# huangzh13/StyleGAN.pytorch

Measured on AMD Instinct MI355X. Metric: img/s full G+D train step, 1024x1024 depth-9 bf16, higher is better.
Workload: dtype bf16; 1 GPU; ffhq1024: StyleGAN 1024x1024, progressive depth index 8, logistic+R1, alpha 0.5, batch 4/GPU, global batch 4; global_batch=4, parallelism=dp1

## Files before the change

include/sgx.h:

```cpp
#ifndef SGX_H
#define SGX_H
#include <stddef.h>
#include <stdint.h>
#ifdef __cplusplus
extern "C" {
#endif

enum { SGX_F32 = 0, SGX_BF16 = 1 };
enum { SGX_ACT_NONE = 0, SGX_ACT_LRELU = 1, SGX_ACT_RELU = 2 };
enum { SGX_EINVAL = -1, SGX_EUNSUPPORTED = -2, SGX_EWORKSPACE = -3 };

int sgx_version(void);
const char* sgx_last_error(void);
int sgx_clear_error(void);
int sgx_stream_wait_stream(void* waiter, void* signaler);
int sgx_selftest_tr16(void* out256, void* stream);

int sgx_prof_start(int mode, int only_of);
int sgx_prof_count(void);
int sgx_prof_get(int i, char* name, int name_cap, float* ms, double* flops, double* bytes, char* desc, int desc_cap);
int sgx_prof_get_launch(int i, unsigned* grid3, unsigned* block3, size_t* lds);

int sgx_conv3x3(const void* x, const void* w, const float* bias, void* y, int B, int H, int W, int Cin, int Cout,
                int act, const void* mask, int dtype, void* stream);
int sgx_conv4x4s2_down(const void* x, const void* w, const float* bias, void* y, int B, int H, int W, int Cin,
                       int Cout, int act, int dtype, void* stream);
int sgx_conv4x4s2_up(const void* x, const void* w, void* y, int B, int H, int W, int Cin, int Cout, int dtype,
                     void* stream);
int sgx_conv_variant(int geo, const void* x, const void* w, const float* bias, void* y, int B, int H, int W, int Cin, int Cout,
                     int act, int dtype, int variant, void* stream);
size_t sgx_conv_splitk_ws_bytes(int geo, int B, int H, int W, int Cin, int Cout, int dtype);
int sgx_conv_splitk(int geo, const void* x, const void* w, const float* bias, void* y, const void* mask, int B, int H, int W, int Cin, int Cout,
                    int act, int dtype, void* ws, size_t ws_bytes, void* stream);

int sgx_conv_config(int geo, int B, int H, int W, int Cin, int Cout, int dtype, int* cfg5);
enum { SGX_PACK_S = 0, SGX_PACK_D = 1, SGX_PACK_U = 2, SGX_PACK_UF = 3 };
int sgx_pack_weight(const float* w, void* fwd, void* adj, int O, int I, int Ipad, int mode, float scale, int dtype,
                    void* stream);
#define SGX_PACK_ROW 10
int sgx_pack_weight_blocks(int O, int Ipad);
int sgx_pack_weight_multi(const void* table, int n, int total_blocks, int dtype, void* stream);
size_t sgx_wgrad_ws_bytes(int taps, int B, int H, int W, int Ck, int Cn);
#define SGX_WGRAD_PLAN_INTS 11
int sgx_wgrad_plan(int taps, int B, int H, int W, int Ck, int Cn, int dtype, size_t ws_bytes, int* out);
int sgx_wgrad3x3_param(const void* x, const void* dy, float* dW, float* db, void* ws, size_t ws_bytes, int B, int H, int W,
                       int Cx, int Cdy, int adjoint, float scale, int O, int I, int accumulate, int dtype, void* stream);
int sgx_wgrad4x4s2_param(const void* fine, const void* coarse, float* dW, float* db, void* ws, size_t ws_bytes, int B, int H,
                         int W, int Cfine, int Ccoarse, int mode, float scale, int O, int I, int accumulate, int dtype,
                         void* stream);

int sgx_bias_act(const void* x, const float* bias, float bscale, void* y, size_t npix, int C, int act, int dtype,
                 void* stream);
int sgx_lrelu_bwd(const void* dy, const void* y, void* dx, size_t n, float slope, float scale, const float* scale_dev, int dtype,
                  void* stream);
int sgx_lrelu_bwd_bits(const void* dy, const void* bits, void* dx, size_t n, float slope, float scale, const float* scale_dev, int dtype,
                       void* stream);
int sgx_conv4x4s2_down_fade_ok(int B, int H, int W, int Cin, int Cout, int dtype);
int sgx_conv4x4s2_down_fade(const void* x, const void* w, const float* bias, const void* resid, float alpha, float beta, const float* ab_dev,
                            void* y, void* bits, int B, int H, int W, int Cin, int Cout, int dtype, void* stream);
int sgx_conv4x4s2_down_fade_rgb(const void* x, const void* w, const float* bias, const float* pimg, const float* wr, float ws, const float* rb,
                                float bs1, float bs2, float alpha, float beta, const float* ab_dev, void* y, void* bits, int B, int H, int W,
                                int Cin, int Cout, int dtype, void* stream);
size_t sgx_fade_rgb_bwd_ws_bytes(size_t npix, int C);
int sgx_fade_rgb_bwd(const void* g, const void* bits, const float* pimg, const float* wr, float ws, float bs, float alpha, float beta,
                     const float* ab_dev, void* gy, float* dwr, float* drb, int acc, float* gpimg, void* wsbuf, size_t ws_bytes, size_t npix, int C,
                     int dtype, void* stream);
int sgx_fade_rgb_bwd_finish(const void* wsbuf, size_t ws_bytes, size_t npix, int C, float ws, float bs, float beta, const float* ab_dev,
                            float* dwr, float* drb, int acc, void* stream);
int sgx_fade_rgb_bwd2(const void* ggy, const float* ggp, const void* bits, const float* wr, float ws, float alpha, float beta, const float* ab_dev,
                      void* out, size_t npix, int C, int dtype, void* stream);
int sgx_axpby(const void* a, const void* b, void* out, float alpha, float beta, size_t n, int dtype, void* stream);
int sgx_axpby_dev(const void* a, const void* b, void* out, const float* alpha_dev, const float* beta_dev, size_t n, int dtype,
                  void* stream);
int sgx_blur3x3(const void* x, void* y, int B, int H, int W, int C, int dtype, void* stream);
int sgx_blur3x3_act(const void* x, const void* z, void* y, int B, int H, int W, int C, int mode, int dtype, void* stream);
int sgx_blur3x3_bits(const void* x, const void* bits, void* y, int B, int H, int W, int C, int mode, int dtype, void* stream);
int sgx_blur_kxk(const void* x, void* y, const float* taps_host, int K, int pad, int B, int IH, int IW, int OH, int OW, int C,
                 int dtype, void* stream);
int sgx_images_u8_to_nhwc(const void* src, void* dst, const int* flip, int B, int H, int W, int src_chw, int dtype, void* stream);
int sgx_pool2(const void* x, void* y, int B, int H, int W, int C, float scale, int dtype, void* stream);
int sgx_up2(const void* x, void* y, int B, int H, int W, int C, float scale, int dtype, void* stream);
int sgx_up2_add(const void* x, const void* a, void* y, int B, int H, int W, int C, float scale, int dtype, void* stream);
size_t sgx_colsum_ws_bytes(size_t npix, int C);
int sgx_colsum(const void* x, float* out, float scale, void* ws, size_t ws_bytes, size_t npix, int C, int dtype,
               void* stream);

int sgx_rgb_in(const float* img, const float* w, int sj, int sc, float wscale, const float* bias, void* y, size_t npix,
               int C, int dtype, void* stream);
int sgx_rgb_out(const void* x, const float* w, int sj, int sc, float wscale, const float* bias, float* img, size_t npix,
                int C, int dtype, void* stream);
int sgx_rgb_in_add(const float* img, const float* w, int sj, int sc, float wscale, const void* add, void* y, size_t npix, int C, int dtype,
                   void* stream);
size_t sgx_rgb_wgrad_ws_bytes(size_t npix, int C);
int sgx_img_in(const float* img, const float* w, int J, int sj, int sc, float wscale, const float* bias, void* y, size_t npix, int C, int dtype,
               void* stream);
int sgx_img_out(const void* x, const float* w, int J, int sj, int sc, float wscale, const float* bias, float* img, size_t npix, int C, int dtype,
                void* stream);
size_t sgx_img_wgrad_ws_bytes(size_t npix, int J, int C);
int sgx_img_wgrad(const float* img, const void* f, float* dw, int J, int sj, int sc, float wscale, void* ws, size_t ws_bytes, size_t npix, int C,
                  int dtype, void* stream);
int sgx_images_u8_to_nhwc_c(const void* src, void* dst, const int* flip, int B, int H, int W, int J, int src_chw, int dtype, void* stream);
int sgx_downsample_fade_rgb(const float* x, float* out, int B, int H, int W, float alpha, float beta, const float* ab_dev, void* stream);
size_t sgx_diffaug_ws_bytes(int B, int H, int W);
int sgx_diffaug(const float* x, float* y, const float* u, int B, int H, int W, int policy_bits, int adjoint, int with_bias, void* ws,
                size_t ws_bytes, void* stream);
int sgx_ada_gates(const float* gu, const float* state, int policy_bits, int* img_bits, int B, void* stream);
int sgx_diffaug_gated(const float* x, float* y, const float* u, const int* img_bits, int B, int H, int W, int policy_bits, int adjoint,
                      int with_bias, void* ws, size_t ws_bytes, void* stream);
int sgx_ada_update(const float* real_logits, int B, float* state, float target, float adjust_per_image, int interval, void* stream);
int sgx_diffaug_blit(const float* x, float* y, const float* u, int u_stride, const int* img_bits, int B, int H, int W, int policy_bits,
                     int adjoint, int with_bias, void* ws, size_t ws_bytes, void* stream);
int sgx_ada_gates_n(const float* gu, int gu_stride, int n_ops, const float* state, int policy_bits, int* img_bits, int B, void* stream);
int sgx_ada_geom_matrix(const float* u, int u_stride, const float* gu, int gu_stride, const float* state, int policy_bits, float* mat, int B,
                        void* stream);
int sgx_ada_geom(const float* x, float* y, const float* mat, int B, int H, int W, int adjoint, void* stream);
int sgx_ada_geom_reflect(const float* x, float* y, const float* mat, int B, int H, int W, int adjoint, void* stream);
#define SGX_ADA_GEOM_REFLECT_PLAN_INTS 6
int sgx_ada_geom_reflect_plan(int B, int H, int W, int adjoint, int aligned, int* out);
int sgx_ada_color_matrix(const float* u, int u_stride, const float* gu, int gu_stride, const float* state, int policy_bits, float* mat, int B,
                         void* stream);
int sgx_ada_color(const float* x, float* y, const float* mat, int B, int H, int W, int adjoint, int with_bias, void* stream);
int sgx_ada_filter_matrix(const float* u, int u_stride, const float* gu, int gu_stride, const float* state, int policy_bits, float* mat, int B,
                          void* stream);
size_t sgx_ada_filter_workspace_bytes(int B, int H, int W);
int sgx_ada_filter(const float* x, float* y, const float* mat, int B, int H, int W, int adjoint, void* ws, size_t ws_bytes, void* stream);
#define SGX_ADA_FILTER_PLAN_INTS 13
int sgx_ada_filter_plan(int B, int H, int W, int adjoint, int aligned, int* out);
int sgx_ada_corrupt_table(const float* u, int u_stride, const float* gu, int gu_stride, const float* state, int policy_bits, int H, int W,
                          float* tab, int B, void* stream);
int sgx_ada_corrupt(const float* x, float* y, const float* tab, int B, int H, int W, int mode, void* stream);
#define SGX_ADA_CORRUPT_PLAN_INTS 5
int sgx_ada_corrupt_plan(int B, int H, int W, int mode, int aligned, int* out);
// ... 102 lines not shown
```

stylegan/pytorch_amd/functional.py:

```python
import contextlib
import functools
import os
import weakref
from collections import namedtuple

import numpy as np
import torch
from torch.autograd import Function
from torch.autograd.function import once_differentiable

from . import native as N

_DATA_GRAD_ONLY = 0


@contextlib.contextmanager
def data_grad_only():
    global _DATA_GRAD_ONLY
    _DATA_GRAD_ONLY += 1
    try:
        yield
    finally:
        _DATA_GRAD_ONLY -= 1

# ... 221 lines not shown
            ent[4][2].add(raw)
    if got is None:
        w = _c(weight.detach())
        if w.dtype != torch.float32:
            raise N.SgxError("parameters must be fp32")
        O, I = w.shape[0], w.shape[1]
        fwd, adj = _pack_alloc(w, sub)
        N.check(N.lib().sgx_pack_weight(N.ptr(w), N.ptr(fwd), N.ptr(adj), O, I, ipad, MODES[mode], float(scale),
                                        N.F32 if dtype == torch.float32 else N.BF16, N.stream()), "sgx_pack_weight")
        got = (fwd, adj)
        ent[2][sub] = got
        ent[4] = _pack_mark()
    return got


def clear_pack_cache():
    for ent in _PACKS.values():
        ent[1], ent[2] = None, {}
    _UPBLUR_PACKS.clear()


_UPBLUR_PACKS = {}


def upblur_pack(weight, mode, scale, ipad, adjoint):
    key = (id(weight), mode, float(scale), int(ipad), bool(adjoint))
    tag = _pack_tag(weight)
    ent = _UPBLUR_PACKS.get(key)
    if ent is not None and ent[0]() is weight and ent[1] == tag:
        raw = N.stream()
        if raw not in ent[3][2] or (not _FAST_FORK and raw != ent[3][1]):
            _stream_of(raw).wait_event(ent[3][0])
            ent[3][2].add(raw)
        return ent[2]
    w = _c(weight.detach())
    if w.dtype != torch.float32 or int(ipad) != w.shape[1]:
        raise N.SgxError("conv+blur composite pack: contiguous fp32 parameter without channel padding expected")
    O, I = w.shape[0], w.shape[1]
    Nn, K = (I, O) if adjoint else (O, I)
    wc = torch.empty(((9 * 4 + 22 * 2) * Nn * K,), dtype=torch.bfloat16, device=w.device)
    N.check(N.lib().sgx_pack_upblur(N.ptr(w), N.ptr(wc), O, I, MODES[mode], int(bool(adjoint)), float(scale) / 16.0, N.stream()), "sgx_pack_upblur")
    _UPBLUR_PACKS[key] = [weakref.ref(weight, lambda _r, k=key: _UPBLUR_PACKS.pop(k, None)), tag, wc, _pack_mark()]
    return wc


@functools.lru_cache(maxsize=None)
def _splitk_ws_bytes(gi, B, H, W, Cin, Cout, dt):
    return int(N.lib().sgx_conv_splitk_ws_bytes(gi, B, H, W, Cin, Cout, dt))


def _conv_launch(geo, x, wq, bias, act, mask=None):
    B, H, W, Cin = x.shape
    taps, Cout, K = wq.shape
    if K != Cin:
        raise N.SgxError(f"conv: weight pack expects {K} input channels, activation has {Cin}")
    L = N.lib()
    gi = "SDU".index(geo)
    wsb = _splitk_ws_bytes(gi, B, H, W, Cin, Cout, N.dt(x))
    if wsb:
        oh, ow = (H, W) if geo == "S" else ((H // 2, W // 2) if geo == "D" else (2 * H, 2 * W))
        y = torch.empty((B, oh, ow, Cout), dtype=x.dtype, device=x.device)
        if mask is not None and (geo != "S" or mask.shape != y.shape or mask.dtype != y.dtype):
            raise N.SgxError("conv: the output mask must have the output's shape and dtype (3x3 geometry)")
        ws = N.workspace(wsb, x.device)
        N.check(L.sgx_conv_splitk(gi, N.ptr(x), N.ptr(wq), N.ptr(bias), N.ptr(y), N.ptr(mask), B, H, W, Cin, Cout, act, N.dt(x), N.ptr(ws), wsb, N.stream()),
                "sgx_conv_splitk")
        return y
    if geo == "S":
        y = torch.empty((B, H, W, Cout), dtype=x.dtype, device=x.device)
        if mask is not None and (mask.shape != y.shape or mask.dtype != y.dtype):
            raise N.SgxError("conv: the output mask must have the output's shape and dtype")
        N.check(L.sgx_conv3x3(N.ptr(x), N.ptr(wq), N.ptr(bias), N.ptr(y), B, H, W, Cin, Cout, act, N.ptr(mask), N.dt(x), N.stream()), "sgx_conv3x3")
    elif geo == "D":
        assert mask is None
        y = torch.empty((B, H // 2, W // 2, Cout), dtype=x.dtype, device=x.device)
        N.check(L.sgx_conv4x4s2_down(N.ptr(x), N.ptr(wq), N.ptr(bias), N.ptr(y), B, H, W, Cin, Cout, act, N.dt(x), N.stream()), "sgx_conv4x4s2_down")
    else:
        assert bias is None and act == 0 and mask is None
        y = torch.empty((B, 2 * H, 2 * W, Cout), dtype=x.dtype, device=x.device)
        N.check(L.sgx_conv4x4s2_up(N.ptr(x), N.ptr(wq), N.ptr(y), B, H, W, Cin, Cout, N.dt(x), N.stream()), "sgx_conv4x4s2_up")
    return y


def _wgrad_param(mode, adjoint, x, gy, weight, scale, want_bias=False, into=None):
    L = N.lib()
    O, I = weight.shape[0], weight.shape[1]
    acc_w = into is not None and into[0] is not None
    acc_b = want_bias and into is not None and into[1] is not None
    dW = into[0] if acc_w else torch.empty((O, I, 3, 3), dtype=torch.float32, device=x.device)
    db = (into[1] if acc_b else torch.empty((O,), dtype=torch.float32, device=x.device)) if want_bias else None
    acc = (1 if acc_w else 0) | (2 if acc_b else 0)
    B = x.shape[0]
    if mode == "S":
        _, H, W, Cx = x.shape
        Cdy = gy.shape[3]
        wsb = L.sgx_wgrad_ws_bytes(9, B, H, W, Cx, Cdy)
        ws = N.workspace(wsb, x.device)
        N.check(L.sgx_wgrad3x3_param(N.ptr(x), N.ptr(gy), N.ptr(dW), N.ptr(db), N.ptr(ws), wsb, B, H, W, Cx, Cdy, int(adjoint),
                                     float(scale), O, I, acc, N.dt(x), N.stream()), "sgx_wgrad3x3_param")
        return dW, db
    launched = ADJ_GEO[mode] if adjoint else FWD_GEO[mode]
    fine, coarse = (x, gy) if launched == "D" else (gy, x)
    _, H, W, Cf = fine.shape
    Cc = coarse.shape[3]
    wsb = L.sgx_wgrad_ws_bytes(16, B, H, W, Cf, Cc)
    ws = N.workspace(wsb, x.device)
    N.check(L.sgx_wgrad4x4s2_param(N.ptr(fine), N.ptr(coarse), N.ptr(dW), N.ptr(db), N.ptr(ws), wsb, B, H, W, Cf, Cc, MODES[mode],
                                   float(scale), O, I, acc, N.dt(x), N.stream()), "sgx_wgrad4x4s2_param")
    return dW, db


class ConvFn(Function):

    @staticmethod
    def forward(ctx, x, weight, bias, mode, scale, ipad, adjoint, act, mask=None, defer_act=False, x_masked=False, stats=None,
                x_pre=None, bits_out=False, x_pre_bits=None):
        x = _c(x)
        fwd, adj = packs(weight, mode, scale, ipad, x.dtype)
        geo = ADJ_GEO[mode] if adjoint else FWD_GEO[mode]
        ctx.cfg = (mode, scale, ipad, adjoint, act, bias is not None, bool(defer_act), bool(x_masked))
        ctx.bias_ref = weakref.ref(bias) if bias is not None else (lambda: None)
        ctx.set_materialize_grads(False)
        if bits_out:
            assert geo == "S" and not adjoint and stats is None
            y, bits = _conv_bits_launch(x, fwd, None if bias is None else _c(bias.detach()), act, mask)
            ctx.mark_non_differentiable(bits)
            ctx.save_for_backward(x, weight, y if (act and not defer_act) else None, mask, x_pre, x_pre_bits)
            return y, bits
        if stats is not None:
            assert geo == "S" and not adjoint and bias is None and act == 0 and mask is None
            y, part = _conv_stats_launch(x, fwd, *stats)
            ctx.mark_non_differentiable(part)
            ctx.save_for_backward(x, weight, None, None, x_pre, x_pre_bits)
            return y, part
        y = _conv_launch(geo, x, adj if adjoint else fwd, None if bias is None else _c(bias.detach()), act, mask)
        ctx.save_for_backward(x, weight, y if (act and not defer_act) else None, mask, x_pre, x_pre_bits)
        return y

    @staticmethod
    def backward(ctx, gy, _gpart=None):
        if gy is None:
            return (None,) * 15
        x, weight, y, mask, x_pre, xb = ctx.saved_tensors[:6]
        mode, scale, ipad, adjoint, act, has_bias, defer_act, x_masked = ctx.cfg
        gy = _c(gy)
        if mask is not None:
            gy = _bcall(LReluBwdFn, gy, mask, 0.2, 1.0)
        if act and not defer_act:
            gy = _bcall(LReluBwdFn, gy, y, 0.2, 1.0)
        gx = gw = gb = None
        if ctx.needs_input_grad[0]:
            if x_pre is not None or xb is not None:
                assert not x_masked
                cout_b = weight.shape[1] if not adjoint else weight.shape[0]
                if xb is not None and conv_upblur_ok(gy, cout_b, mode, not adjoint):
                    gx = _bcall(ConvBlurFn, gy, weight, mode, scale, ipad, not adjoint, None, xb)
                elif x_pre is not None and conv_blur_ok(gy, cout_b, mode, not adjoint, has_mask_tensor=True):
                    gx = _bcall(ConvBlurFn, gy, weight, mode, scale, ipad, not adjoint, x_pre)
                else:
                    gx = _bcall(BlurMaskFn, _bcall(ConvFn, gy, weight, None, mode, scale, ipad, not adjoint, 0), x_pre, xb)
            else:
                gx = _bcall(ConvFn, gy, weight, None, mode, scale, ipad, not adjoint, 0, x if x_masked else None, False, False)
        if not _DATA_GRAD_ONLY:
            want_b = has_bias and ctx.needs_input_grad[2]
            fuse_b = want_b and ctx.needs_input_grad[1] and not adjoint and mode in ("S", "D")
            if ctx.needs_input_grad[1] and _ACCUM_PARAM_GRADS and weight.is_leaf and not torch.is_grad_enabled():
                bias = ctx.bias_ref() if fuse_b else None
                if fuse_b and (bias is None or not bias.is_leaf):
                    fuse_b, bias = False, None
                dW, db = _param_grads(mode, adjoint, _c(x), gy, weight, scale, fuse_b, (weight.grad, bias.grad if fuse_b else None))
                if weight.grad is None:
                    weight.grad = dW
                if fuse_b:
                    if bias.grad is None:
                        bias.grad = db
                    want_b = False
                if GRAD_NOTE is not None:
                    GRAD_NOTE(weight)
                    if fuse_b:
                        GRAD_NOTE(bias)
            elif ctx.needs_input_grad[1]:
                gw, gb = _bcall(WgradFn, x, gy, weight, mode, scale, adjoint, fuse_b)
            if want_b and not fuse_b:
                gb = _bcall(ColSumFn, gy, 1.0)
        return gx, gw, gb, None, None, None, None, None, None, None, None, None, None, None, None


# ... 1985 lines not shown
```

stylegan/pytorch_amd/native.py:

```python
import ctypes
import os
import subprocess
import threading

import torch

_HERE = os.path.dirname(os.path.abspath(__file__))
LIB_PATH = os.environ.get("SGX_HIP_LIB") or os.path.join(_HERE, "libsgx_hip.so")
CSRC = os.path.join(_HERE, "csrc")

F32, BF16 = 0, 1
ACT_NONE, ACT_LRELU, ACT_RELU = 0, 1, 2
EPI_ACT, EPI_NORM = 1, 2
PACK_S, PACK_D, PACK_U, PACK_UF = 0, 1, 2, 3

_lib = None
_lock = threading.Lock()

c_void_p, c_int, c_float, c_size_t = ctypes.c_void_p, ctypes.c_int, ctypes.c_float, ctypes.c_size_t
P, I, F, Z = c_void_p, c_int, c_float, c_size_t

SIGNATURES = {
    "sgx_version": (I, []),
    "sgx_last_error": (ctypes.c_char_p, []),
    "sgx_clear_error": (I, []),
    "sgx_stream_wait_stream": (I, [P, P]),
    "sgx_conv3x3": (I, [P, P, P, P, I, I, I, I, I, I, P, I, P]),
    "sgx_conv_variant": (I, [I, P, P, P, P, I, I, I, I, I, I, I, I, P]),
    "sgx_conv4x4s2_down": (I, [P, P, P, P, I, I, I, I, I, I, I, P]),
    "sgx_conv4x4s2_up": (I, [P, P, P, I, I, I, I, I, I, P]),
    "sgx_wgrad_ws_bytes": (Z, [I, I, I, I, I, I]),
    "sgx_wgrad_plan": (I, [I, I, I, I, I, I, I, Z, P]),
    "sgx_images_u8_to_nhwc": (I, [P, P, P, I, I, I, I, I, P]),
    "sgx_selftest_tr16": (I, [P, P]),
    "sgx_conv_splitk_ws_bytes": (Z, [I, I, I, I, I, I, I]),
    "sgx_conv_splitk": (I, [I, P, P, P, P, P, I, I, I, I, I, I, I, P, Z, P]),
    "sgx_conv_config": (I, [I, I, I, I, I, I, I, P]),
    "sgx_prof_start": (I, [I, I]),
    "sgx_prof_count": (I, []),
    "sgx_prof_get": (I, [I, P, I, P, P, P, P, I]),
    "sgx_prof_get_launch": (I, [I, P, P, P]),
    "sgx_pack_weight": (I, [P, P, P, I, I, I, I, F, I, P]),
    "sgx_pack_weight_multi": (I, [P, I, I, I, P]),
    "sgx_pack_weight_blocks": (I, [I, I]),
    "sgx_wgrad3x3_param": (I, [P, P, P, P, P, Z, I, I, I, I, I, I, F, I, I, I, I, P]),
    "sgx_wgrad4x4s2_param": (I, [P, P, P, P, P, Z, I, I, I, I, I, I, F, I, I, I, I, P]),
    "sgx_bias_act": (I, [P, P, F, P, Z, I, I, I, P]),
    "sgx_lrelu_bwd": (I, [P, P, P, Z, F, F, P, I, P]),
    "sgx_lrelu_bwd_bits": (I, [P, P, P, Z, F, F, P, I, P]),
    "sgx_conv4x4s2_down_fade_ok": (I, [I, I, I, I, I, I]),
    "sgx_conv4x4s2_down_fade": (I, [P, P, P, P, F, F, P, P, P, I, I, I, I, I, I, P]),
    "sgx_conv4x4s2_down_fade_rgb": (I, [P, P, P, P, P, F, P, F, F, F, F, P, P, P, I, I, I, I, I, I, P]),
    "sgx_fade_rgb_bwd_ws_bytes": (Z, [Z, I]),
    "sgx_fade_rgb_bwd": (I, [P, P, P, P, F, F, F, F, P, P, P, P, I, P, P, Z, Z, I, I, P]),
    "sgx_fade_rgb_bwd_finish": (I, [P, Z, Z, I, F, F, F, P, P, P, I, P]),
    "sgx_fade_rgb_bwd2": (I, [P, P, P, P, F, F, F, P, P, Z, I, I, P]),
    "sgx_axpby": (I, [P, P, P, F, F, Z, I, P]),
    "sgx_axpby_dev": (I, [P, P, P, P, P, Z, I, P]),
    "sgx_blur3x3": (I, [P, P, I, I, I, I, I, P]),
    "sgx_blur3x3_act": (I, [P, P, P, I, I, I, I, I, I, P]),
    "sgx_blur_kxk": (I, [P, P, P, I, I, I, I, I, I, I, I, I, P]),
    "sgx_pool2": (I, [P, P, I, I, I, I, F, I, P]),
    "sgx_up2": (I, [P, P, I, I, I, I, F, I, P]),
    "sgx_up2_add": (I, [P, P, P, I, I, I, I, F, I, P]),
    "sgx_colsum_ws_bytes": (Z, [Z, I]),
    "sgx_colsum": (I, [P, P, F, P, Z, Z, I, I, P]),
    "sgx_rgb_in": (I, [P, P, I, I, F, P, P, Z, I, I, P]),
    "sgx_rgb_in_add": (I, [P, P, I, I, F, P, P, Z, I, I, P]),
    "sgx_rgb_out": (I, [P, P, I, I, F, P, P, Z, I, I, P]),
    "sgx_img_in": (I, [P, P, I, I, I, F, P, P, Z, I, I, P]),
    "sgx_img_out": (I, [P, P, I, I, I, F, P, P, Z, I, I, P]),
    "sgx_img_wgrad_ws_bytes": (Z, [Z, I, I]),
    "sgx_img_wgrad": (I, [P, P, P, I, I, I, F, P, Z, Z, I, I, P]),
    "sgx_images_u8_to_nhwc_c": (I, [P, P, P, I, I, I, I, I, I, P]),
    "sgx_downsample_fade_rgb": (I, [P, P, I, I, I, F, F, P, P]),
    "sgx_diffaug_ws_bytes": (Z, [I, I, I]),
    "sgx_diffaug": (I, [P, P, P, I, I, I, I, I, I, P, Z, P]),
    "sgx_ada_gates": (I, [P, P, I, P, I, P]),
    "sgx_diffaug_gated": (I, [P, P, P, P, I, I, I, I, I, I, P, Z, P]),
    "sgx_ada_update": (I, [P, I, P, F, F, I, P]),
    "sgx_diffaug_blit": (I, [P, P, P, I, P, I, I, I, I, I, I, P, Z, P]),
    "sgx_ada_gates_n": (I, [P, I, I, P, I, P, I, P]),
    "sgx_ada_geom_matrix": (I, [P, I, P, I, P, I, P, I, P]),
    "sgx_ada_geom": (I, [P, P, P, I, I, I, I, P]),
    "sgx_ada_geom_reflect": (I, [P, P, P, I, I, I, I, P]),
    "sgx_ada_geom_reflect_plan": (I, [I, I, I, I, I, P]),
    "sgx_ada_color_matrix": (I, [P, I, P, I, P, I, P, I, P]),
    "sgx_ada_color": (I, [P, P, P, I, I, I, I, I, P]),
    "sgx_ada_filter_matrix": (I, [P, I, P, I, P, I, P, I, P]),
    "sgx_ada_filter_workspace_bytes": (Z, [I, I, I]),
    "sgx_ada_filter": (I, [P, P, P, I, I, I, I, P, Z, P]),
    "sgx_ada_filter_plan": (I, [I, I, I, I, I, P]),
    "sgx_ada_corrupt_table": (I, [P, I, P, I, P, I, I, I, P, I, P]),
    "sgx_ada_corrupt": (I, [P, P, P, I, I, I, I, P]),
    "sgx_ada_corrupt_plan": (I, [I, I, I, I, I, P]),
    "sgx_aug_plan": (I, [I, I, I, I, I, I, I, I, P]),
    "sgx_rgb_out_fade": (I, [P, P, I, I, F, P, P, F, F, P, P, I, I, I, I, I, P]),
    "sgx_rgb_wgrad_ws_bytes": (Z, [Z, I]),
    "sgx_rgb_wgrad": (I, [P, P, P, I, I, F, P, Z, Z, I, I, P]),
    "sgx_gepi_ws_bytes": (Z, [I, I, I]),
    "sgx_gepi_fwd": (I, [P, P, P, P, P, P, P, P, P, Z, P, I, I, I, I, I, I, P]),
    "sgx_gepi_stats": (I, [P, P, P, P, P, P, P, Z, P, I, I, I, I, I, I, P]),
    "sgx_gepi_plan": (I, [I, I, I, I, I, I, I, P]),
    "sgx_rgb_out_epi": (I, [P, P, P, P, P, P, P, P, I, I, F, P, P, F, F, P, P, I, I, I, I, I, P]),
    "sgx_rgb_wgrad_epi_ws_bytes": (Z, [I, I, I]),
    "sgx_rgb_wgrad_epi": (I, [P, P, P, P, P, P, P, P, P, P, I, I, F, F, P, Z, I, I, I, I, P]),
    "sgx_blur3x3_stats_nparts": (I, [I, I, I, I, I]),
    "sgx_conv3x3_stats_nparts": (I, [I, I, I, I, I, I]),
    "sgx_conv3x3_signbits_ok": (I, [I, I, I, I, I, I]),
    "sgx_conv3x3_signbits": (I, [P, P, P, P, P, I, I, I, I, I, I, P, I, P]),
    "sgx_blur3x3_bits": (I, [P, P, P, I, I, I, I, I, I, P]),
    "sgx_conv4x4s2_up_blur_ok": (I, [I, I, I, I, I, I]),
    "sgx_conv4x4s2_up_blur": (I, [P, P, P, P, I, I, I, I, I, I, P]),
    "sgx_conv4x4s2_up_blur_bits": (I, [P, P, P, P, I, I, I, I, I, I, P]),
    "sgx_pack_upblur": (I, [P, P, I, I, I, I, F, P]),
    "sgx_conv_upblur_ok": (I, [I, I, I, I, I, I]),
    "sgx_conv_upblur": (I, [P, P, P, P, I, I, I, I, I, I, P]),
    "sgx_rgbconv_ok": (I, [I, I, I, I, I]),
    "sgx_rgbconv_pack": (I, [P, F, P, F, P, F, P, P, I, P]),
    "sgx_rgbconv_fwd": (I, [P, P, P, P, P, I, I, I, I, I, I, I, P]),
    "sgx_rgbconv_tune": (I, [I, I, I]),
    "sgx_rgbconv_dgrad": (I, [P, P, P, I, I, I, I, I, P]),
    "sgx_rgbconv_plan": (I, [I, I, I, I, I, I, P]),
    "sgx_rgbconv_wgrad_ws_bytes": (Z, [I, I, I, I]),
    "sgx_rgbconv_wgrad": (I, [P, P, I, P, F, P, F, P, F, P, P, P, P, I, P, Z, I, I, I, I, I, P]),
    "sgx_conv3x3_stats": (I, [P, P, P, P, P, P, P, Z, I, I, I, I, I, I, P]),
    "sgx_blur3x3_stats": (I, [P, P, P, P, P, P, Z, I, I, I, I, I, I, P]),
    "sgx_gepi_bwd": (I, [P, P, P, P, P, P, P, P, P, P, P, P, P, Z, I, I, I, I, I, P]),
    "sgx_pixelnorm_fwd": (I, [P, P, I, I, P]),
# ... 242 lines not shown
```

Before: 299.5 img/s.

## Add single-pass low-resolution weight-gradient kernels for 3x3 and 4x4s2 convolutions

```diff
diff --git a/include/sgx.h b/include/sgx.h
--- a/include/sgx.h
+++ b/include/sgx.h
@@ -48,6 +48,12 @@
 int sgx_wgrad4x4s2_param(const void* fine, const void* coarse, float* dW, float* db, void* ws, size_t ws_bytes, int B, int H,
                          int W, int Cfine, int Ccoarse, int mode, float scale, int O, int I, int accumulate, int dtype,
                          void* stream);
+int sgx_wgrad_lowres_ok(int taps, int B, int H, int W, int Ck, int Cn, int dtype);
+int sgx_wgrad3x3_param_lowres(const void* x, const void* dy, float* dW, float* db, void* ws, size_t ws_bytes, int B, int H, int W,
+                              int Cx, int Cdy, int adjoint, float scale, int O, int I, int accumulate, int dtype, void* stream);
+int sgx_wgrad4x4s2_param_lowres(const void* fine, const void* coarse, float* dW, float* db, void* ws, size_t ws_bytes, int B, int H,
+                                int W, int Cfine, int Ccoarse, int mode, float scale, int O, int I, int accumulate, int dtype,
+                                void* stream);
 
 int sgx_bias_act(const void* x, const float* bias, float bscale, void* y, size_t npix, int C, int act, int dtype,
                  void* stream);
diff --git a/stylegan/pytorch_amd/csrc/wgrad3.hip b/stylegan/pytorch_amd/csrc/wgrad3.hip
--- /dev/null
+++ b/stylegan/pytorch_amd/csrc/wgrad3.hip
@@ -0,0 +1,397 @@
+#include "common.h"
+
+typedef __attribute__((ext_vector_type(16))) float f32x16;
+
+__device__ __attribute__((aligned(64))) const unsigned wg3_zero_page[16] = {0, 0, 0, 0, 0, 0, 0, 0, 0, 0, 0, 0, 0, 0, 0, 0};
+
+__device__ __forceinline__ void wg3_glds16(const void* g, char* lds_wave_base) {
+    __builtin_amdgcn_global_load_lds((const __attribute__((address_space(1))) void*)g,
+                                     (__attribute__((address_space(3))) void*)lds_wave_base, 16, 0, 0);
+}
+__device__ __forceinline__ s16x4 wg3_tr16(const char* p) {
+    return __builtin_amdgcn_ds_read_tr16_b64_v4i16((s16x4 __attribute__((address_space(3)))*)(p));
+}
+__device__ __forceinline__ bf16x8 wg3_frag(const char* lo, const char* hi) {
+    typedef __attribute__((ext_vector_type(8))) short s16x8;
+    const s16x4 vl = wg3_tr16(lo), vh = wg3_tr16(hi);
+    const s16x8 v = __builtin_shufflevector(vl, vh, 0, 1, 2, 3, 4, 5, 6, 7);
+    return __builtin_bit_cast(bf16x8, v);
+}
+__device__ __forceinline__ bf16x8 wg3_ones() {
+    typedef __attribute__((ext_vector_type(8))) short s16x8;
+    const s16x8 v = {0x3f80, 0x3f80, 0x3f80, 0x3f80, 0x3f80, 0x3f80, 0x3f80, 0x3f80};
+    return __builtin_bit_cast(bf16x8, v);
+}
+
+__device__ __forceinline__ int wg3_swz(int pix, int h) { return h ^ ((pix >> 1) & 1); }
+
+struct Wg3Args {
+    const bf16_t* kside; const bf16_t* nside; float* dw; float* db;
+    int B, Hn, Wn, Ck, Cn;
+    int nct_k, nblk;
+    int O, I, mode, transposed, flip_t, accumulate; float scale;
+};
+
+__device__ __forceinline__ int wg3_block(int nblk) {
+    const int bid = blockIdx.x;
+    return (nblk & 7) == 0 ? (bid & 7) * (nblk >> 3) + (bid >> 3) : bid;
+}
+
+template <int W>
+__global__ __launch_bounds__(512) void wgrad_lowres_s_kernel(Wg3Args a) {
+    constexpr int NP = 256, SR = NP / W, PW = W + 2;
+    constexpr int A_BYTES = NP * 128, A_INSTR = NP / 8;
+    constexpr int B_PIX = SR * PW, B_INSTR = (B_PIX + 7) / 8, B_BYTES = B_INSTR * 1024;
+    constexpr int STAGE = A_BYTES + B_BYTES, NINSTR = A_INSTR + B_INSTR, NPI = (NINSTR + 7) / 8;
+    constexpr int NSEG = 2, KS = NP / 16 / NSEG;
+    constexpr int KP = 65;
+    static_assert(NP % W == 0 && W % 8 == 0, "whole rows; both reads of a lane in one row");
+    extern __shared__ __attribute__((aligned(1024))) char smem[];
+
+    const int tid = threadIdx.x, lane = tid & 63, l31 = lane & 31, hi = lane >> 5;
+    const int wave = __builtin_amdgcn_readfirstlane(tid >> 6);
+    const int bid = wg3_block(a.nblk);
+    const int dy = bid % 3, ct = bid / 3;
+    const int n0 = (ct / a.nct_k) * 64, k0 = (ct % a.nct_k) * 64;
+    const int rows = a.B * a.Hn, npix = rows * W;
+    const int nsteps = (npix + NP - 1) / NP;
+
+    int rel[NPI], pos[NPI];
+#pragma unroll
+    for (int jj = 0; jj < NPI; ++jj) {
+        const int ii = jj * 8 + wave, c16 = (lane & 3) * 8, half = (lane >> 2) & 1;
+        rel[jj] = 0; pos[jj] = -1;
+        if (ii < A_INSTR) {
+            const int pix = ii * 8 + (lane >> 3);
+            rel[jj] = pix * a.Cn + wg3_swz(pix, half) * 32 + c16;
+            pos[jj] = pix;
+        } else if (ii < NINSTR) {
+            const int pix = (ii - A_INSTR) * 8 + (lane >> 3);
+            if (pix < B_PIX) {
+                const int pr = pix / PW, pc = pix % PW;
+                rel[jj] = (pr * W + pc - 1) * a.Ck + wg3_swz(pix, half) * 32 + c16;
+                pos[jj] = (pr << 8) | pc;
+            }
+        }
+    }
+    const unsigned long long zaddr = reinterpret_cast<unsigned long long>(wg3_zero_page) + (lane & 3) * 16;
+    const unsigned long long na = reinterpret_cast<unsigned long long>(a.nside), ka = reinterpret_cast<unsigned long long>(a.kside);
+    auto issue = [&](int step, char* buf) {
+        const long long aoff = (long long)step * NP * a.Cn + n0;
+        const long long boff = ((long long)(step * SR + dy - 1) * W) * a.Ck + k0;
+#pragma unroll
+        for (int jj = 0; jj < NPI; ++jj) {
+            const int ii = jj * 8 + wave;
+            if (ii < NINSTR) {
+                const bool isb = ii >= A_INSTR;
+                const int pp = pos[jj];
+                bool ok;
+                if (!isb) ok = step * NP + pp < npix;
+                else {
+                    const int g = step * SR + (pp >> 8), y = g % a.Hn + dy - 1, x = (pp & 255) - 1;
+                    ok = (pp >= 0) & (g < rows) & ((unsigned)y < (unsigned)a.Hn) & ((unsigned)x < (unsigned)W);
+                }
+                const unsigned long long m = ok ? ~0ull : 0ull;
+                const unsigned long long pa = (isb ? ka : na) + (unsigned long long)(((isb ? boff : aoff) + rel[jj]) * 2);
+                wg3_glds16(reinterpret_cast<const void*>(zaddr + ((pa - zaddr) & m)), buf + ii * 1024);
+            }
+        }
+    };
+
+    const int nb = (wave >> 1) & 1, kb = wave & 1, seg = wave >> 2;
+    const int g16 = lane >> 4, i16 = lane & 15;
+    const int lp = (g16 >> 1) * 8 + (i16 >> 2);
+    const int lane_c = (g16 & 1) * 32 + (i16 & 3) * 8;
+    const bool do_bias = a.db != nullptr && k0 == 0 && dy == 0 && kb == 0;
+
+    f32x16 acc[3], bacc;
+#pragma unroll
+    for (int r = 0; r < 16; ++r) {
+        bacc[r] = 0.f;
+#pragma unroll
+        for (int t = 0; t < 3; ++t) acc[t][r] = 0.f;
+    }
+    const bf16x8 ones = wg3_ones();
+
+    if (nsteps > 0) issue(0, smem);
+    for (int step = 0; step < nsteps; ++step) {
+        const char* cur = smem + (step & 1) * STAGE;
+        __syncthreads();
+        if (step + 1 < nsteps) issue(step + 1, smem + ((step + 1) & 1) * STAGE);
+#pragma unroll
+        for (int s = 0; s < KS; ++s) {
+            const int p = (seg * KS + s) * 16 + lp;
+            const int q = (p / W) * PW + p % W;
+            const char* ap = cur + lane_c + p * 128 + wg3_swz(p, nb) * 64;
+            const bf16x8 af = wg3_frag(ap, ap + 512);
+            if (do_bias) bacc = __builtin_amdgcn_mfma_f32_32x32x16_bf16(af, ones, bacc, 0, 0, 0);
+#pragma unroll
+            for (int dx = 0; dx < 3; ++dx) {
+                const char* bp = cur + A_BYTES + lane_c + (q + dx) * 128 + wg3_swz(q + dx, kb) * 64;
+                const bf16x8 bf = wg3_frag(bp, bp + 512);
+                acc[dx] = __builtin_amdgcn_mfma_f32_32x32x16_bf16(af, bf, acc[dx], 0, 0, 0);
+            }
+        }
+    }
+
+    float* accl = reinterpret_cast<float*>(smem);
+    float* bl = accl + 3 * 64 * KP;
+    __syncthreads();
+    for (int r = NSEG - 1; r >= 0; --r) {
+        if (seg == r) {
+#pragma unroll
+            for (int g = 0; g < 4; ++g)
+#pragma unroll
+                for (int j = 0; j < 4; ++j) {
+                        const int nl = nb * 32 + 8 * g + 4 * hi + j;
+#pragma unroll
+                        for (int dx = 0; dx < 3; ++dx) {
+                            float* q = accl + (dx * 64 + nl) * KP + kb * 32 + l31;
+                            *q = r == NSEG - 1 ? acc[dx][4 * g + j] : acc[dx][4 * g + j] + *q;
+                        }
+                        if (do_bias && l31 == 0) {
+                            const float v = r == NSEG - 1 ? bacc[4 * g + j] : bacc[4 * g + j] + bl[nl];
+                            if (r) bl[nl] = v;
+                            else {
+                                float* d = a.db + n0 + nl;
+                                *d = (a.accumulate & 2) ? *d + v : v;
+                            }
+                        }
+                    }
+        }
+        __syncthreads();
+    }
+    const float c = a.scale;
+    for (int idx = tid; idx < 64 * 64; idx += 512) {
+        const int fast = idx & 63, slow = idx >> 6;
+        const int nl = a.transposed ? fast : slow, kl = a.transposed ? slow : fast;
+        const int n = n0 + nl, k = k0 + kl;
+        const int o = a.transposed ? k : n, i = a.transposed ? n : k;
+        if (i >= a.I || o >= a.O) continue;
+        float* d = a.dw + ((size_t)o * a.I + i) * 9;
+#pragma unroll
+        for (int dx = 0; dx < 3; ++dx) {
+            const int t = dy * 3 + dx, tap = a.flip_t ? 8 - t : t;
+            const float v = accl[(dx * 64 + nl) * KP + kl];
+            d[tap] = (a.accumulate & 1) ? d[tap] + c * v : c * v;
+        }
+    }
+}
+
+template <int TW, int TH, int NB>
+__global__ __launch_bounds__(512) void wgrad_lowres_d_kernel(Wg3Args a) {
+    constexpr int PH = TH + 1, PW = TW + 1, PPIX = PH * PW, BAND = TH * TW, NP = NB * BAND;
+    constexpr int A_PLANE = NP * 64, A_INSTR = NP / 16;
+    constexpr int B_PIX = NB * PPIX, B_INSTR = (B_PIX * 64 + 1023) / 1024, B_PLANE = B_INSTR * 1024;
+    constexpr int STAGE = 2 * A_PLANE + 4 * B_PLANE, NINSTR = 2 * A_INSTR + 4 * B_INSTR, NPI = (NINSTR + 7) / 8;
+    constexpr int KS = NP / 16;
+    constexpr int KP = 33;
+    static_assert(NP % 16 == 0 && BAND % 16 == 0 && TW % 4 == 0, "a K-step inside one band, a read's 4 pixels inside one row");
+    extern __shared__ __attribute__((aligned(1024))) char smem[];
+
+    const int tid = threadIdx.x, lane = tid & 63, l31 = lane & 31, hi = lane >> 5;
+    const int wave = __builtin_amdgcn_readfirstlane(tid >> 6);
+    const int ct = wg3_block(a.nblk);
+    const int n0 = (ct / a.nct_k) * 64, k0 = (ct % a.nct_k) * 32;
+    const int Hk = 2 * a.Hn, Wk = 2 * TW;
+    const int bpi = a.Hn / TH, nbands = a.B * bpi, npix = nbands * BAND;
+    const int nsteps = (nbands + NB - 1) / NB;
+
+    int rel[NPI], posy[NPI], posx[NPI];
+#pragma unroll
+    for (int jj = 0; jj < NPI; ++jj) {
+        const int ii = jj * 8 + wave, c16 = (lane & 3) * 8;
+        rel[jj] = 0; posy[jj] = -1; posx[jj] = 0;
+        if (ii < 2 * A_INSTR) {
+            const int plane = ii / A_INSTR, pix = (ii % A_INSTR) * 16 + (lane >> 2);
+            rel[jj] = pix * a.Cn + plane * 32 + c16;
+            posy[jj] = 0; posx[jj] = pix;
+        } else if (ii < NINSTR) {
+            const int j = ii - 2 * A_INSTR, ph = j / B_INSTR, pix = (j % B_INSTR) * 16 + (lane >> 2);
+            if (pix < B_PIX) {
+                const int bd = pix / PPIX, q = pix % PPIX, pr = q / PW, pc = q % PW, fy = 2 * pr - (ph >> 1), fx = 2 * pc - (ph & 1);
+                rel[jj] = ((bd * 2 * TH + fy) * Wk + fx) * a.Ck + c16;
+                posy[jj] = (fy + 1) | (bd << 16); posx[jj] = fx;
+            }
+        }
+    }
+    const unsigned long long zaddr = reinterpret_cast<unsigned long long>(wg3_zero_page) + (lane & 3) * 16;
+    const unsigned long long na = reinterpret_cast<unsigned long long>(a.nside), ka = reinterpret_cast<unsigned long long>(a.kside);
+    auto issue = [&](int step, char* buf) {
+        const long long aoff = (long long)step * NP * a.Cn + n0;
+        const long long boff = ((long long)step * NB * 2 * TH * Wk) * a.Ck + k0;
+#pragma unroll
+        for (int jj = 0; jj < NPI; ++jj) {
+            const int ii = jj * 8 + wave;
+            if (ii < NINSTR) {
+                const bool isb = ii >= 2 * A_INSTR;
+                bool ok;
+                if (!isb) ok = step * NP + posx[jj] < npix;
+                else {
+                    const int band = step * NB + (posy[jj] >> 16), gy = 2 * (band % bpi) * TH + (posy[jj] & 0xffff) - 1;
+                    ok = (posy[jj] >= 0) & (band < nbands) & ((unsigned)gy < (unsigned)Hk) & ((unsigned)posx[jj] < (unsigned)Wk);
+                }
+                const unsigned long long m = ok ? ~0ull : 0ull;
+                const unsigned long long pa = (isb ? ka : na) + (unsigned long long)(((isb ? boff : aoff) + rel[jj]) * 2);
+                wg3_glds16(reinterpret_cast<const void*>(zaddr + ((pa - zaddr) & m)), buf + ii * 1024);
+            }
+        }
+    };
+
+    const int ph = wave & 3, nb = wave >> 2, py = ph >> 1, px = ph & 1;
+    const int g16 = lane >> 4, i16 = lane & 15;
+    const int lp = (g16 >> 1) * 8 + (i16 >> 2);
+    const int lane_c = (g16 & 1) * 32 + (i16 & 3) * 8;
+    const int b_off = 2 * A_PLANE + ph * B_PLANE + lane_c;
+    const bool do_bias = a.db != nullptr && k0 == 0 && ph == 0;
+    auto patch = [&](int p) { return ((p / BAND) * PPIX + ((p % BAND) / TW) * PW + p % TW) * 64; };
+
+    f32x16 acc[2][2], bacc;
+#pragma unroll
+    for (int r = 0; r < 16; ++r) {
+        bacc[r] = 0.f;
+#pragma unroll
+        for (int e = 0; e < 2; ++e)
+#pragma unroll
+            for (int f = 0; f < 2; ++f) acc[e][f][r] = 0.f;
+    }
+    const bf16x8 ones = wg3_ones();
+
+    if (nsteps > 0) issue(0, smem);
+    for (int step = 0; step < nsteps; ++step) {
+        const char* cur = smem + (step & 1) * STAGE;
+        __syncthreads();
+        if (step + 1 < nsteps) issue(step + 1, smem + ((step + 1) & 1) * STAGE);
+#pragma unroll
+        for (int s = 0; s < KS; ++s) {
+            const int p = s * 16 + lp;
+            const char* ap = cur + nb * A_PLANE + p * 64 + lane_c;
+            const bf16x8 af = wg3_frag(ap, ap + 256);
+            if (do_bias) bacc = __builtin_amdgcn_mfma_f32_32x32x16_bf16(af, ones, bacc, 0, 0, 0);
+            const char* blo = cur + b_off + patch(p);
+            const char* bhi = cur + b_off + patch(p + 4);
+#pragma unroll
+            for (int e = 0; e < 2; ++e)
+#pragma unroll
+                for (int f = 0; f < 2; ++f) {
+                    const bf16x8 bf = wg3_frag(blo + (e * PW + f) * 64, bhi + (e * PW + f) * 64);
+                    acc[e][f] = __builtin_amdgcn_mfma_f32_32x32x16_bf16(af, bf, acc[e][f], 0, 0, 0);
+                }
+        }
+    }
+
+    float* accl = reinterpret_cast<float*>(smem);
+    __syncthreads();
+#pragma unroll
+    for (int e = 0; e < 2; ++e)
+#pragma unroll
+        for (int f = 0; f < 2; ++f) {
+            const int t = (2 * e + 1 - py) * 4 + (2 * f + 1 - px);
+#pragma unroll
+            for (int g = 0; g < 4; ++g)
+#pragma unroll
+                for (int j = 0; j < 4; ++j) accl[(t * 64 + nb * 32 + 8 * g + 4 * hi + j) * KP + l31] = acc[e][f][4 * g + j];
+        }
+    if (do_bias && l31 == 0) {
+#pragma unroll
+        for (int g = 0; g < 4; ++g)
+#pragma unroll
+            for (int j = 0; j < 4; ++j) {
+                float* d = a.db + n0 + nb * 32 + 8 * g + 4 * hi + j;
+                *d = (a.accumulate & 2) ? *d + bacc[4 * g + j] : bacc[4 * g + j];
+            }
+    }
+    __syncthreads();
+    const float c = a.scale * (a.mode == SGX_PACK_D ? 0.25f : 1.f);
+    for (int idx = tid; idx < 64 * 32; idx += 512) {
+        const int nl = a.transposed ? idx & 63 : idx >> 5, kl = a.transposed ? idx >> 6 : idx & 31;
+        const int n = n0 + nl, k = k0 + kl;
+        const int o = a.transposed ? k : n, i = a.transposed ? n : k;
+        if (i >= a.I || o >= a.O) continue;
+        float v[16];
+#pragma unroll
+        for (int t = 0; t < 16; ++t) v[t] = accl[(t * 64 + nl) * KP + kl];
+        float* d = a.dw + ((size_t)o * a.I + i) * 9;
+#pragma unroll
+        for (int y = 0; y < 3; ++y)
+#pragma unroll
+            for (int x = 0; x < 3; ++x) {
+                const float sum = (v[y * 4 + x] + v[y * 4 + x + 1]) + (v[(y + 1) * 4 + x] + v[(y + 1) * 4 + x + 1]);
+                const int tap = y * 3 + x, q = a.mode == SGX_PACK_UF ? 8 - tap : tap;
+                d[q] = (a.accumulate & 1) ? d[q] + c * sum : c * sum;
+            }
+    }
+}
+
+static constexpr int WG3_MAX_PIX = 8192;
+static int wg3_th(int wn) { return wn == 8 ? 8 : 4; }
+extern "C" int sgx_wgrad_lowres_ok(int taps, int B, int H, int W, int Ck, int Cn, int dtype) {
+    if (dtype != SGX_BF16 || (taps != 9 && taps != 16) || B < 1 || H < 1 || W < 1) return 0;
+    if (Ck < 64 || Cn < 64 || Ck % 64 || Cn % 64) return 0;
+    if ((long)B * H * W > WG3_MAX_PIX) return 0;
+    if (taps == 9) return W == 8 || W == 16 || W == 32;
+    if (H % 2 || W % 2) return 0;
+    const int hn = H / 2, wn = W / 2;
+    return (wn == 4 || wn == 8 || wn == 16) && hn % wg3_th(wn) == 0;
+}
+
+template <int W>
+static int wg3_launch_s(const Wg3Args& a, hipStream_t st) {
+    constexpr int NP = 256, BP = ((NP / W * (W + 2) + 7) / 8) * 1024;
+    constexpr int OPER = 2 * (NP * 128 + BP), FOLD = (3 * 64 * 65 + 64) * 4;
+    constexpr int LDS = OPER > FOLD ? OPER : FOLD;
+    static_assert(LDS <= 160 * 1024, "LDS budget");
+    sgx_lds_opt_in<wgrad_lowres_s_kernel<W>>(LDS);
+    hipLaunchKernelGGL(wgrad_lowres_s_kernel<W>, dim3((unsigned)a.nblk), dim3(512), LDS, st, a);
+    SGX_LAUNCH_CHECK("wgrad_lowres_s_kernel");
+    return 0;
+}
+template <int TW, int TH, int NB>
+static int wg3_launch_d(const Wg3Args& a, hipStream_t st) {
+    constexpr int NP = NB * TH * TW, BP = ((NB * (TH + 1) * (TW + 1) * 64 + 1023) / 1024) * 1024;
+    constexpr int OPER = 2 * (2 * NP * 64 + 4 * BP), FOLD = (16 * 64 * 33 + 64) * 4;
+    constexpr int LDS = OPER > FOLD ? OPER : FOLD;
+    static_assert(LDS <= 160 * 1024, "LDS budget");
+    sgx_lds_opt_in<wgrad_lowres_d_kernel<TW, TH, NB>>(LDS);
+    hipLaunchKernelGGL((wgrad_lowres_d_kernel<TW, TH, NB>), dim3((unsigned)a.nblk), dim3(512), LDS, st, a);
+    SGX_LAUNCH_CHECK("wgrad_lowres_d_kernel");
+    return 0;
+}
+
+extern "C" int sgx_wgrad3x3_param_lowres(const void* x, const void* dy, float* dW, float* db, void* ws, size_t ws_bytes, int B, int H, int W,
+                                         int Cx, int Cdy, int adjoint, float scale, int O, int I, int accumulate, int dtype, void* stream) {
+    (void)ws; (void)ws_bytes;
+    const int Ip = adjoint ? Cdy : Cx;
+    SGX_REQUIRE(x && dy && dW, SGX_EINVAL, "wgrad3x3_param_lowres: NULL argument");
+    SGX_REQUIRE(!db || !adjoint, SGX_EINVAL, "wgrad3x3_param_lowres: bias gradient asked of the adjoint launch");
+    SGX_REQUIRE((adjoint ? Cx : Cdy) == O && Ip >= I, SGX_EINVAL, "wgrad3x3_param_lowres: channel mismatch (Cx=%d Cdy=%d O=%d I=%d adj=%d)", Cx, Cdy, O, I, adjoint);
+    SGX_REQUIRE(sgx_wgrad_lowres_ok(9, B, H, W, Cx, Cdy, dtype), SGX_EUNSUPPORTED,
+                "wgrad3x3_param_lowres: shape not taken (B%d %dx%d %dx%d dtype %d), see sgx_wgrad_lowres_ok", B, H, W, Cx, Cdy, dtype);
+    Wg3Args a{static_cast<const bf16_t*>(x), static_cast<const bf16_t*>(dy), dW, db, B, H, W, Cx, Cdy, Cx / 64, (Cdy / 64) * (Cx / 64) * 3,
+              O, I, SGX_PACK_S, adjoint, adjoint, accumulate, scale};
+    SGX_NOTE(2.0 * 9 * Cx * Cdy * B * H * W, 2.0 * B * H * W * (Cx + Cdy), "wgradS-lowres B%d %dx%d %dx%d", B, H, W, Cx, Cdy);
+    hipStream_t st = (hipStream_t)stream;
+    return W == 8 ? wg3_launch_s<8>(a, st) : W == 16 ? wg3_launch_s<16>(a, st) : wg3_launch_s<32>(a, st);
+}
+
+extern "C" int sgx_wgrad4x4s2_param_lowres(const void* fine, const void* coarse, float* dW, float* db, void* ws, size_t ws_bytes, int B, int H,
+                                           int W, int Cfine, int Ccoarse, int mode, float scale, int O, int I, int accumulate, int dtype,
+                                           void* stream) {
+    (void)ws; (void)ws_bytes;
+    SGX_REQUIRE(fine && coarse && dW, SGX_EINVAL, "wgrad4x4s2_param_lowres: NULL argument");
+    SGX_REQUIRE(H % 2 == 0 && W % 2 == 0, SGX_EINVAL, "wgrad4x4s2_param_lowres: odd fine size");
+    SGX_REQUIRE(mode == SGX_PACK_D || mode == SGX_PACK_U || mode == SGX_PACK_UF, SGX_EINVAL, "wgrad4x4s2_param_lowres: bad mode %d", mode);
+    const int transposed = mode != SGX_PACK_D;
+    SGX_REQUIRE(!db || !transposed, SGX_EINVAL, "wgrad4x4s2_param_lowres: bias gradient only for mode D (dy is the coarse side)");
+    SGX_REQUIRE(transposed ? (Ccoarse == I && Cfine == O) : (Ccoarse == O && Cfine == I), SGX_EINVAL,
+                "wgrad4x4s2_param_lowres: channel mismatch (fine %d coarse %d O %d I %d mode %d)", Cfine, Ccoarse, O, I, mode);
+    SGX_REQUIRE(sgx_wgrad_lowres_ok(16, B, H, W, Cfine, Ccoarse, dtype), SGX_EUNSUPPORTED,
+                "wgrad4x4s2_param_lowres: shape not taken (B%d fine %dx%d %dx%d dtype %d), see sgx_wgrad_lowres_ok", B, H, W, Cfine, Ccoarse, dtype);
+    Wg3Args a{static_cast<const bf16_t*>(fine), static_cast<const bf16_t*>(coarse), dW, db, B, H / 2, W / 2, Cfine, Ccoarse, Cfine / 32,
+              (Ccoarse / 64) * (Cfine / 32), O, I, mode, transposed, 0, accumulate, scale};
+    SGX_NOTE(2.0 * 16 * Cfine * Ccoarse * B * (H / 2) * (W / 2), 2.0 * B * H * W * (Cfine + Ccoarse / 4.0), "wgradD-lowres B%d fine%dx%d %dx%d", B, H, W,
+             Cfine, Ccoarse);
+    hipStream_t st = (hipStream_t)stream;
+    const int wn = W / 2;
+    return wn == 4 ? wg3_launch_d<4, 4, 8>(a, st) : wn == 8 ? wg3_launch_d<8, 8, 2>(a, st) : wg3_launch_d<16, 4, 2>(a, st);
+}
diff --git a/stylegan/pytorch_amd/functional.py b/stylegan/pytorch_amd/functional.py
--- a/stylegan/pytorch_amd/functional.py
+++ b/stylegan/pytorch_amd/functional.py
@@ -327,6 +327,19 @@
     return y
 
 
+WGRAD_LOWRES = int(os.environ.get("SGX_WGRAD_LOWRES", "1") or 0)
+
+
+def wgrad_lowres_routed(taps, B, H, W, Ck, Cn):
+    return taps == 9 and W == 32 and Ck >= 512 and Cn >= 512 and B * H * W >= 4096
+
+
+def _wgrad_lowres(L, taps, B, H, W, Ck, Cn, dtype):
+    if not WGRAD_LOWRES or not L.sgx_wgrad_lowres_ok(taps, B, H, W, Ck, Cn, dtype):
+        return False
+    return WGRAD_LOWRES >= 2 or wgrad_lowres_routed(taps, B, H, W, Ck, Cn)
+
+
 def _wgrad_param(mode, adjoint, x, gy, weight, scale, want_bias=False, into=None):
     L = N.lib()
     O, I = weight.shape[0], weight.shape[1]
@@ -339,6 +352,10 @@
     if mode == "S":
         _, H, W, Cx = x.shape
         Cdy = gy.shape[3]
+        if _wgrad_lowres(L, 9, B, H, W, Cx, Cdy, N.dt(x)):
+            N.check(L.sgx_wgrad3x3_param_lowres(N.ptr(x), N.ptr(gy), N.ptr(dW), N.ptr(db), None, 0, B, H, W, Cx, Cdy, int(adjoint),
+                                                float(scale), O, I, acc, N.dt(x), N.stream()), "sgx_wgrad3x3_param_lowres")
+            return dW, db
         wsb = L.sgx_wgrad_ws_bytes(9, B, H, W, Cx, Cdy)
         ws = N.workspace(wsb, x.device)
         N.check(L.sgx_wgrad3x3_param(N.ptr(x), N.ptr(gy), N.ptr(dW), N.ptr(db), N.ptr(ws), wsb, B, H, W, Cx, Cdy, int(adjoint),
@@ -348,6 +365,10 @@
     fine, coarse = (x, gy) if launched == "D" else (gy, x)
     _, H, W, Cf = fine.shape
     Cc = coarse.shape[3]
+    if _wgrad_lowres(L, 16, B, H, W, Cf, Cc, N.dt(x)):
+        N.check(L.sgx_wgrad4x4s2_param_lowres(N.ptr(fine), N.ptr(coarse), N.ptr(dW), N.ptr(db), None, 0, B, H, W, Cf, Cc, MODES[mode],
+                                              float(scale), O, I, acc, N.dt(x), N.stream()), "sgx_wgrad4x4s2_param_lowres")
+        return dW, db
     wsb = L.sgx_wgrad_ws_bytes(16, B, H, W, Cf, Cc)
     ws = N.workspace(wsb, x.device)
     N.check(L.sgx_wgrad4x4s2_param(N.ptr(fine), N.ptr(coarse), N.ptr(dW), N.ptr(db), N.ptr(ws), wsb, B, H, W, Cf, Cc, MODES[mode],
diff --git a/stylegan/pytorch_amd/native.py b/stylegan/pytorch_amd/native.py
--- a/stylegan/pytorch_amd/native.py
+++ b/stylegan/pytorch_amd/native.py
@@ -45,6 +45,9 @@
     "sgx_pack_weight_blocks": (I, [I, I]),
     "sgx_wgrad3x3_param": (I, [P, P, P, P, P, Z, I, I, I, I, I, I, F, I, I, I, I, P]),
     "sgx_wgrad4x4s2_param": (I, [P, P, P, P, P, Z, I, I, I, I, I, I, F, I, I, I, I, P]),
+    "sgx_wgrad_lowres_ok": (I, [I, I, I, I, I, I, I]),
+    "sgx_wgrad3x3_param_lowres": (I, [P, P, P, P, P, Z, I, I, I, I, I, I, F, I, I, I, I, P]),
+    "sgx_wgrad4x4s2_param_lowres": (I, [P, P, P, P, P, Z, I, I, I, I, I, I, F, I, I, I, I, P]),
     "sgx_bias_act": (I, [P, P, F, P, Z, I, I, I, P]),
     "sgx_lrelu_bwd": (I, [P, P, P, Z, F, F, P, I, P]),
     "sgx_lrelu_bwd_bits": (I, [P, P, P, Z, F, F, P, I, P]),
```

Result: no change. 299.2 img/s, median of 2 (-0.1%).
